# AlexandreRouma/SDRPlusPlus

Measured on NVIDIA H100. Metric: complex IQ MSamples/s through FFT + 8-VFO WFM chain, higher is better.
Workload: dtype f32

## Files before the change

sdrplusplus_b200/csrc/api.cpp:

```cpp
#include "../../include/b200dsp.h"
#include "engine.h"
#include <chrono>
#include <map>
#include <cmath>
#include <cstdio>
#include <cstring>
#include <cstdlib>
#include <algorithm>

using namespace b200;

static int g_device = -1;

static int ensure_device() {
    int n = 0;
    cudaError_t e = cudaGetDeviceCount(&n);
    if (e != cudaSuccess || n <= 0) {
        set_error("no usable CUDA device (%s): libb200dsp has no CPU fallback", e == cudaSuccess ? "0 devices" : cudaGetErrorString(e));
        cudaGetLastError();
        return B200_ENODEV;
    }
    if (g_device < 0) { g_device = 0; }
    B200_CK(cudaSetDevice(g_device));
    return 0;
// ... 170 lines not shown
    Scheduler sch_pre;
    DevBuf pp[FE_SLOTS];
    DevBuf dc_state, dc_segA, dc_segB;
    int max_eff = 0;
};

static float fe_ingest_scale(const b200_fe* fe, int fmt) {
    if (fmt == B200_FMT_CS16) { return fe->scale16; }
    if (fmt == B200_FMT_CS8) { return fe->scale8; }
    return 0.0f;
}

static int fe_alloc_fft(b200_fe* fe) {
    int rc;
    if ((rc = fe->frame.alloc((size_t)fe->fft.nz * sizeof(float2)))) { return rc; }
    long long interval = (long long)fe->fft.nz + fe->skip;
    fe->max_lines = (int)(fe->max_eff / interval) + 2;
    return fe->lines.alloc((size_t)fe->max_lines * fe->fft.size * sizeof(float));
}

extern "C" b200_fe* b200_fe_create(double samplerate, int max_chunk) {
    if (ensure_device()) { return nullptr; }
    if (samplerate <= 0 || max_chunk < 1) { set_error("bad samplerate/max_chunk"); return nullptr; }
    b200_fe* fe = new b200_fe;
    fe->fs = samplerate;
    fe->fs_eff = samplerate;
    fe->max_chunk = max_chunk;
    fe->max_eff = max_chunk;
    int lo = 0, hi = 0;
    cudaDeviceGetStreamPriorityRange(&lo, &hi);
    int pt = 2, pm = 1, pf = 0;
    if (const char* e = getenv("B200_STREAM_PRIO")) { sscanf(e, "%d,%d,%d", &pt, &pm, &pf); }
    if (const char* e = getenv("B200_FFT_SERIAL")) { fe->fft_serial = atoi(e); }
    if (const char* e = getenv("B200_FFT_CTA")) { kernels_set_fft_cta(atoi(e)); }
    auto prio = [&](int level) { int p = lo - level; return p < hi ? hi : p; };
    bool ok = cudaStreamCreateWithPriority(&fe->own_stream, cudaStreamNonBlocking, prio(pm)) == cudaSuccess &&
              cudaStreamCreateWithFlags(&fe->copy_stream, cudaStreamNonBlocking) == cudaSuccess &&
              cudaStreamCreateWithPriority(&fe->fft_stream, cudaStreamNonBlocking, prio(pf)) == cudaSuccess &&
              cudaStreamCreateWithPriority(&fe->tail_stream, cudaStreamNonBlocking, prio(pt)) == cudaSuccess &&
              cudaStreamCreateWithFlags(&fe->join_stream, cudaStreamNonBlocking) == cudaSuccess &&
              cudaEventCreateWithFlags(&fe->ev_lines_free, cudaEventDisableTiming) == cudaSuccess &&
              cudaEventCreateWithFlags(&fe->ev_fft_go, cudaEventDisableTiming) == cudaSuccess &&
              cudaEventCreateWithFlags(&fe->ev_fft_done, cudaEventDisableTiming) == cudaSuccess;
    for (int i = 0; i < FE_SLOTS && ok; i++) {
        ok = cudaEventCreateWithFlags(&fe->ev_h2d[i], cudaEventDisableTiming) == cudaSuccess &&
             cudaEventCreateWithFlags(&fe->ev_compute[i], cudaEventDisableTiming) == cudaSuccess &&
             cudaEventCreateWithFlags(&fe->ev_tail_done[i], cudaEventDisableTiming) == cudaSuccess &&
             cudaEventCreateWithFlags(&fe->ev_out[i], cudaEventDisableTiming) == cudaSuccess;
    }
    if (!ok || fe->sch.init_raw()) {
        if (ok) {} else { cuda_fail(cudaGetLastError(), "stream/event creation"); }
        b200_fe_destroy(fe);
        return nullptr;
    }
    fe->sch.stream = fe->own_stream;
    fe->sch.fuse.on = true;
    kernels_set_xd_tma_stages(2);
    kernels_set_xd_tma_diag(0);
    {
        int dev = 0, sms = 0;
        if (cudaGetDevice(&dev) == cudaSuccess && cudaDeviceGetAttribute(&sms, cudaDevAttrMultiProcessorCount, dev) == cudaSuccess && sms > 0) {
            fe->sch.sm_count = sms;
        }
    }
    if (fe->sch.enable_overlap(fe->tail_stream)) { b200_fe_destroy(fe); return nullptr; }
    return fe;
}
// ... 202 lines not shown
    if (!strcmp(key, "graphs")) { return (long long)fe->sch.graphs.size(); }
    if (!strcmp(key, "host_ns_stage1")) { return fe->sch.host_ns[0]; }
    if (!strcmp(key, "host_ns_tail")) { return fe->sch.host_ns[1]; }
    return -1;
}
extern "C" int b200_fe_set_option(b200_fe* fe, const char* key, int value) {
    if (!fe || !key) { set_error("null argument"); return B200_EINVAL; }
    if (!strcmp(key, "s1")) { fe->sch.s1_variant = value; return 0; }
    if (!strcmp(key, "overlap")) {
        if (b200_fe_vfo_count(fe) > 0) { set_error("'overlap' must be chosen before VFOs are added"); return B200_ESTATE; }
        if (cudaDeviceSynchronize() != cudaSuccess) { return cuda_fail(cudaGetLastError(), "sync"); }
        fe->sch.tail_stream = value ? fe->tail_stream : nullptr;
        return 0;
    }
    if (!strcmp(key, "pair")) { fe->sch.pair_conjugates = value != 0; return 0; }
    if (!strcmp(key, "fft_async")) { fe->fft_async = value != 0; return 0; }
    if (!strcmp(key, "s1_mt")) { kernels_set_xd_tile(value); return 0; }
    if (!strcmp(key, "s1_cps")) { kernels_set_xd_cps(value); return 0; }
    if (!strcmp(key, "s1_stages")) { kernels_set_xd_tma_stages(value); return 0; }
    if (!strcmp(key, "s1_diag")) { kernels_set_xd_tma_diag(value); return 0; }
    if (!strcmp(key, "s1_ctas")) { kernels_set_xd_tma_ctas(value); return 0; }
    if (!strcmp(key, "tails") || !strncmp(key, "ft_", 3)) {
        if (b200_fe_vfo_count(fe) > 0) { set_error("'%s' must be chosen before VFOs are added", key); return B200_ESTATE; }
        if (!strcmp(key, "tails")) { kernels_set_tail_variant(value >= 1 ? 1 : 0); fe->sch.fuse.on = value >= 2; return 0; }
        if (!strcmp(key, "ft_ob")) { fe->sch.fuse.ob_force = value; return 0; }
        if (!strcmp(key, "ft_obmax")) { fe->sch.fuse.ob_max = value; return 0; }
        if (!strcmp(key, "ft_smem_kb")) { fe->sch.fuse.smem_limit = value * 1024; return 0; }
        if (!strcmp(key, "ft_threads")) { fe->sch.fuse.threads = value; return 0; }
        if (!strcmp(key, "ft_direct")) { fe->sch.fuse.direct = value != 0; return 0; }
        if (!strcmp(key, "ft_prereg")) { fe->sch.fuse.pre_reg = value; return 0; }
        if (!strcmp(key, "ft_regall")) { fe->sch.fuse.reg_all = value != 0; return 0; }
    }
    if (!strcmp(key, "fft")) { kernels_set_fft_variant(value); return 0; }
    if (!strcmp(key, "fft_cta")) { kernels_set_fft_cta(value); return 0; }
    if (!strcmp(key, "host_direct")) { fe->host_direct = value; return 0; }
    if (!strcmp(key, "inflight")) {
        if (value < 1 || value > FE_SLOTS) { set_error("inflight: 1 ... %d", FE_SLOTS); return B200_EINVAL; }
        fe->max_inflight = value;
        return 0;
    }
    if (!strcmp(key, "fft_serial")) { fe->fft_serial = value; return 0; }
    if (!strcmp(key, "graph")) { fe->sch.graph_tails = value; if (value == 0) { fe->sch.drop_graphs(); } return 0; }
    if (!strcmp(key, "graph_max_count")) { fe->sch.graph_max_count = value; return 0; }
    if (!strcmp(key, "pdl")) { kernels_set_pdl(value); fe->sch.drop_graphs(); return 0; }
    if (!strcmp(key, "tail_split")) { fe->sch.tail_split = value; fe->sch.drop_graphs(); return 0; }
    if (!strcmp(key, "time_s1")) { fe->sch.time_s1 = value != 0; for (auto& t : fe->sch.timers) { t.used = 0; } return 0; }
    set_error("unknown option %s", key);
    return B200_EINVAL;
}

extern "C" int b200_fe_s1_stats(b200_fe* fe, double* ms_total, int* launches) {
    if (!fe || !ms_total || !launches) { set_error("null argument"); return B200_EINVAL; }
    return fe->sch.s1_stats(ms_total, launches);
}
extern "C" int b200_fe_group_stats(b200_fe* fe, int group, double* ms_total, int* launches) {
    if (!fe || !ms_total || !launches) { set_error("null argument"); return B200_EINVAL; }
    return fe->sch.group_stats(group, ms_total, launches);
}

extern "C" int b200_fe_reset(b200_fe* fe) {
    if (!fe) { set_error("null fe"); return B200_EINVAL; }
    std::lock_guard<std::mutex> lck(fe->mtx);
    B200_CK(cudaDeviceSynchronize());
    for (auto& v : fe->vfos) {
        if (v->used) { v->chain.reset_state(); }
    }
    int rc = fe->sch.reset_raw();
// ... 35 lines not shown
                v->cfg.bandwidth = v->new_bw;
            }
            v->pend_bw = false;
        }
    }
}

static int fe_fft_chunk(b200_fe* fe, const void* dptr, int fmt, int count, int* nlines) {
    *nlines = 0;
    if (!fe->fft_on) { fe->pos += (unsigned long long)count; return 0; }
    const unsigned long long pos = fe->pos, end = pos + (unsigned long long)count;
    const unsigned long long nz = (unsigned long long)fe->fft.nz, interval = nz + (unsigned long long)fe->skip;
    const int bps = bytes_per_sample(fmt);
    const float isc = fe_ingest_scale(fe, fmt);
    fe->fft.plan.in_scale = isc;
    cudaStream_t main_s = fe->sch.stream;
    const bool async = fe->fft_async || fe->sch.tail_stream != nullptr;
    float* const lines_base = fe->lines_override ? fe->lines_override : fe->lines.as<float>();
    cudaStream_t s = async ? fe->fft_stream : main_s;
    bool forked = false;
    cudaEvent_t t_fft = nullptr;
    auto fork = [&]() -> int {
        if (async && !forked) {
            B200_CK(cudaEventRecord(fe->ev_fft_go, main_s));
            B200_CK(cudaStreamWaitEvent(s, fe->ev_fft_go, 0));
            if (fe->lines_busy) { B200_CK(cudaStreamWaitEvent(s, fe->ev_lines_free, 0)); }
            trace_mark("fft start", s);
            t_fft = fe->sch.timer_begin(2, s);
            forked = true;
        }
        return 0;
    };
    int rc = 0;
    if (fe->fstart < pos) {
        const unsigned long long fend = fe->fstart + nz;
        const unsigned long long lo = pos, hi = std::min(fend, end);
        if (hi > lo) {
            if ((rc = fork())) { return rc; }
            cudaError_t e = launch_convert_cf32(dptr, fmt, fe->frame.as<float2>() + (size_t)(lo - fe->fstart), (int)(hi - lo), isc, s);
            if (e != cudaSuccess) { return cuda_fail(e, "launch_convert_cf32"); }
            fe->sch.launches++;
        }
        if (fend <= end) {
            if ((rc = fork())) { return rc; }
            int nl = 0;
            cudaError_t e = launch_fft_frame(fe->fft.plan, fe->frame.p, FMT_CF32, fe->fft.work.as<float2>(), lines_base, nullptr, s, &nl);
            if (e != cudaSuccess) { return cuda_fail(e, "launch_fft_frame"); }
            fe->sch.launches += nl;
            (*nlines)++;
            fe->fstart += interval;
        }
    }
    if (fe->fstart >= pos && fe->fstart + nz <= end) {
        int nb = (int)((end - fe->fstart - nz) / interval) + 1;
        if (*nlines + nb > fe->max_lines) { set_error("FFT line buffer overflow"); return B200_ECAP; }
        if ((rc = fork())) { return rc; }
        const char* src = (const char*)dptr + (size_t)(fe->fstart - pos) * bps;
        int nl = 0;
        cudaError_t e = launch_fft_frames(fe->fft.plan, src, fmt, fe->fft.work.as<float2>(),
                                          lines_base + (size_t)(*nlines) * fe->fft.size, nullptr, s, &nl, nb,
                                          (long long)interval * bps);
        if (e != cudaSuccess) { return cuda_fail(e, "launch_fft_frames"); }
        fe->sch.launches += nl;
        *nlines += nb;
        fe->fstart += interval * (unsigned long long)nb;
    }
    if (fe->fstart < end && fe->fstart >= pos) {
        const unsigned long long lo = fe->fstart, hi = end;
        if (hi > lo) {
            if ((rc = fork())) { return rc; }
            const char* src = (const char*)dptr + (size_t)(lo - pos) * bps;
            cudaError_t e = launch_convert_cf32(src, fmt, fe->frame.as<float2>(), (int)(hi - lo), isc, s);
            if (e != cudaSuccess) { return cuda_fail(e, "launch_convert_cf32"); }
            fe->sch.launches++;
        }
    }
    if (forked) {
        if (t_fft) { B200_CK(cudaEventRecord(t_fft, s)); }
        trace_mark("fft done", s);
        B200_CK(cudaEventRecord(fe->ev_fft_done, s));
        fe->fft_join_pending = true;
        if (fe->fft_serial && s != main_s) { B200_CK(cudaStreamWaitEvent(main_s, fe->ev_fft_done, 0)); }
    }
    fe->pos = end;
    return 0;
}

extern "C" int b200_fe_submit(b200_fe* fe, const void* iq, int count, int in_fmt, int in_mem, b200_outputs* out) {
    if (!fe || !out || (count > 0 && !iq)) { set_error("null argument"); return B200_EINVAL; }
    if (count < 0 || count > fe->max_chunk) { set_error("count %d exceeds max_chunk %d", count, fe->max_chunk); return B200_ECAP; }
    if (in_fmt < 0 || in_fmt > 2) { set_error("bad input format"); return B200_EINVAL; }
    if (fe->nsub - fe->nwait >= (unsigned long long)fe->max_inflight) { set_error("%d chunks already in flight: call b200_fe_wait", fe->max_inflight); return B200_ESTATE; }
    std::lock_guard<std::mutex> lck(fe->mtx);
    const long long hp0 = host_clock_ns();
    apply_pending(fe);
    const int slot = (int)(fe->nsub % FE_SLOTS);
    cudaStream_t s = fe->sch.stream;
    const size_t in_bytes = (size_t)count * bytes_per_sample(in_fmt);
    std::vector<Chain*> chains;
    std::vector<int> ids;
    for (size_t i = 0; i < fe->vfos.size(); i++) {
        if (fe->vfos[i]->used) { chains.push_back(&fe->vfos[i]->chain); ids.push_back((int)i); }
    }
    const int ecount = (fe->decim > 1) ? fe->pre.peek(count) : count;
    if (ecount < 0) { set_error("input decimator is not a FIR cascade"); return B200_ESTATE; }
// ... 951 lines not shown
```

sdrplusplus_b200/csrc/fft_reg.cuh:

```cuda
#pragma once

__device__ constexpr float FR_COS[16] = { 1.000000000e+00f, 9.807852804e-01f, 9.238795325e-01f, 8.314696123e-01f, 7.071067812e-01f, 5.555702330e-01f,
                                          3.826834324e-01f, 1.950903220e-01f, 0.0f, -1.950903220e-01f, -3.826834324e-01f, -5.555702330e-01f,
                                          -7.071067812e-01f, -8.314696123e-01f, -9.238795325e-01f, -9.807852804e-01f };
__device__ constexpr float FR_SIN[16] = { 0.000000000e+00f, 1.950903220e-01f, 3.826834324e-01f, 5.555702330e-01f, 7.071067812e-01f, 8.314696123e-01f,
                                          9.238795325e-01f, 9.807852804e-01f, 1.0f, 9.807852804e-01f, 9.238795325e-01f, 8.314696123e-01f,
                                          7.071067812e-01f, 5.555702330e-01f, 3.826834324e-01f, 1.950903220e-01f };

template <int R, int K>
__device__ __forceinline__ float2 fr_mul_w(float2 v) {
    constexpr int k32 = K * (32 / R);
    if constexpr (k32 == 0) { return v; }
    else if constexpr (k32 == 8) { return make_float2(v.y, -v.x); }
    else if constexpr (k32 == 4) { return make_float2((v.x + v.y) * RSQRT2, (v.y - v.x) * RSQRT2); }
    else if constexpr (k32 == 12) { return make_float2((v.y - v.x) * RSQRT2, -(v.x + v.y) * RSQRT2); }
    else {
        constexpr float c = FR_COS[k32], s = FR_SIN[k32];
        return make_float2(fmaf(v.y, s, v.x * c), fmaf(-v.x, s, v.y * c));
    }
}
template <int R, int H, int I>
__device__ __forceinline__ void fr_stage(float2 (&a)[R]) {
    constexpr int blk = I / H, j = I % H, i0 = blk * 2 * H + j;
    const float2 u = a[i0], v = a[i0 + H];
// ... 14 lines not shown
    static constexpr int n = RA * RB;
    static constexpr int TP = RA > RB ? RA : RB;
    static constexpr int crow = RB + 1;
    static constexpr int pitch = ((RA * crow + 13) / 16) * 16 + 2;
};

template <int RA, int RB>
__device__ __forceinline__ void fr_transform(float2 (&v)[RA > RB ? RA : RB], float2* ex, int t, const float2* __restrict__ tw, int twsh) {
    using G = FrGeom<RA, RB>;
    if (t < RB) {
        float2 a[RA];
#pragma unroll
        for (int i = 0; i < RA; i++) { a[i] = v[i]; }
        fr_dft<RA>(a);
#pragma unroll
        for (int c = 0; c < RA; c++) {
            float2 y = a[fr_brev<RA>(c)];
            if (c > 0) { y = cmulf(y, __ldg(tw + ((size_t)(t * c) << twsh))); }
            ex[c * G::crow + t] = y;
        }
    }
    __syncthreads();
    if (t < RA) {
        float2 b[RB];
#pragma unroll
        for (int i = 0; i < RB; i++) { b[i] = ex[t * G::crow + i]; }
        fr_dft<RB>(b);
#pragma unroll
        for (int i = 0; i < RB; i++) { v[i] = b[i]; }
    }
}

template <int FMT, int RA, int RB, int C, int MINB>
__global__ void __launch_bounds__(C * FrGeom<RA, RB>::TP, MINB) k_fftr_p1(const __grid_constant__ FftPlanDev pl, const void* __restrict__ src0,
                                                                    float2* __restrict__ work0, long long src_stride_bytes) {
    using G = FrGeom<RA, RB>;
    extern __shared__ __align__(16) float2 smem[];
    const int N2 = pl.N2;
    const void* src = reinterpret_cast<const char*>(src0) + (size_t)blockIdx.y * src_stride_bytes;
    float2* work = work0 + (size_t)blockIdx.y * pl.N;
    const int col = threadIdx.x % C, t = threadIdx.x / C;
    const int n2 = blockIdx.x * C + col;
    float2 v[G::TP];
    if (t < RB) {
#pragma unroll
        for (int a = 0; a < RA; a++) { v[a] = load_windowed<FMT>(pl, src, (a * RB + t) * N2 + n2); }
    }
    fr_transform<RA, RB>(v, smem + col * G::pitch, t, pl.tw, pl.logTW - pl.logN1);
    if (t < RA) {
        const int s = pl.logN - pl.logTW;
        const unsigned msk = (1u << s) - 1u;
#pragma unroll
        for (int d = 0; d < RB; d++) {
            const int k1 = t + RA * d;
            const unsigned e = (unsigned)k1 * (unsigned)n2;
            const float2 w = cmulf(__ldg(pl.tw + (e >> s)), __ldg(pl.tw_fine + (e & msk)));
            work[(size_t)k1 * N2 + n2] = cmulf(v[fr_brev<RB>(d)], w);
        }
    }
}

template <int RA, int RB, int R>
__global__ void __launch_bounds__(R * FrGeom<RA, RB>::TP) k_fftr_p2(const __grid_constant__ FftPlanDev pl, const float2* __restrict__ work0,
                                                                    float* __restrict__ out_db0) {
    using G = FrGeom<RA, RB>;
    extern __shared__ __align__(16) float2 smem[];
    const int N1 = pl.N1, N2 = pl.N2;
    const float2* work = work0 + (size_t)blockIdx.y * pl.N;
    float* out_db = out_db0 + (size_t)blockIdx.y * pl.N;
    const int t = threadIdx.x % G::TP, row = threadIdx.x / G::TP;
    const int r0 = blockIdx.x * R;
    float2 v[G::TP];
    if (t < RB) {
        const float2* __restrict__ p = work + (size_t)(r0 + row) * N2 + t;
#pragma unroll
        for (int a = 0; a < RA; a++) { v[a] = __ldg(p + a * RB); }
    }
    fr_transform<RA, RB>(v, smem + row * G::pitch, t, pl.tw, pl.logTW - pl.logN2);
    __syncthreads();
// ... 13 lines not shown
```

sdrplusplus_b200/csrc/kernels.cu:

```cuda
#include "kernels.cuh"
#include <unordered_map>
#include <mutex>
#include <math.h>
#include <string.h>
#include <algorithm>

template <int FMT>
__device__ __forceinline__ float2 load_iq(const void* __restrict__ p, long long i, float sc) {
    if (FMT == FMT_CF32) {
        return __ldg(reinterpret_cast<const float2*>(p) + i);
    }
    else if (FMT == FMT_CS16) {
        short2 v = __ldg(reinterpret_cast<const short2*>(p) + i);
        return make_float2((float)v.x * sc, (float)v.y * sc);
    }
    else {
        char2 v = __ldg(reinterpret_cast<const char2*>(p) + i);
        return make_float2((float)v.x * sc, (float)v.y * sc);
    }
}

template <int FMT>
__device__ __forceinline__ float2 load_x(const XdParams& p, long long i) {
    if (i >= 0) {
// ... 432 lines not shown
    }
    else if (lognb == 1) {
        const int per = n >> 1, logper = logn - 1;
        for (int t = tid; t < per * C; t += nthr) {
            int c, bi;
            if (BATCH_INNER) { c = t & (C - 1); bi = t >> logC; }
            else { bi = t & (per - 1); c = t >> logper; }
            const int base = bi * 2;
            float2 a0 = s[fft_addr<BATCH_INNER>(base + 0, c, C, pitch)];
            float2 a1 = s[fft_addr<BATCH_INNER>(base + 1, c, C, pitch)];
            s[fft_addr<BATCH_INNER>(base + 0, c, C, pitch)] = cadd(a0, a1);
            s[fft_addr<BATCH_INNER>(base + 1, c, C, pitch)] = csub(a0, a1);
        }
        __syncthreads();
    }
}

__device__ __forceinline__ int bitrev(int k, int bits) { return (int)(__brev((unsigned)k) >> (32 - bits)); }

__device__ __forceinline__ float power_db(float2 X, float normFactSq) {
    float m2 = (X.x * X.x + X.y * X.y) * normFactSq;
    float l = log2f(m2);
    if (isinf(l)) { l = copysignf(127.0f, l); }
    return l * 3.01029995663981209120f;
}

template <int FMT>
__device__ __forceinline__ float2 load_windowed(const FftPlanDev& pl, const void* __restrict__ src, int n) {
    if (n >= pl.nz) { return make_float2(0.0f, 0.0f); }
    float2 x = load_iq<FMT>(src, n, pl.in_scale);
    float w = __ldg(pl.window + n);
    return make_float2(x.x * w, x.y * w);
}

template <int FMT>
__global__ void __launch_bounds__(512) k_fft_single(const __grid_constant__ FftPlanDev pl, const void* __restrict__ src0,
                                                      float* __restrict__ out_db0, float2* __restrict__ out_raw,
                                                      long long src_stride_bytes) {
    extern __shared__ __align__(16) float2 smem[];
    const int N = pl.N;
    const void* src = reinterpret_cast<const char*>(src0) + (size_t)blockIdx.y * src_stride_bytes;
    float* out_db = out_db0 + (size_t)blockIdx.y * N;
#pragma unroll 4
    for (int i = threadIdx.x; i < N; i += blockDim.x) { smem[padf(i)] = load_windowed<FMT>(pl, src, i); }
    __syncthreads();
    fft_dif_smem<false>(smem, pl.logN, 1, N, pl.tw, pl.logTW);
    const float nf = 1.0f / ((float)N * (float)N);
    for (int k = threadIdx.x; k < N; k += blockDim.x) {
        float2 X = smem[padf(bitrev(k, pl.logN))];
        out_db[k] = power_db(X, nf);
        if (out_raw) { out_raw[k] = X; }
    }
}

template <int FMT>
__global__ void __launch_bounds__(512) k_fft_p1(const __grid_constant__ FftPlanDev pl, const void* __restrict__ src0,
                                                  float2* __restrict__ work0, int C, long long src_stride_bytes) {
    extern __shared__ __align__(16) float2 smem[];
    const int N1 = pl.N1, N2 = pl.N2;
    const void* src = reinterpret_cast<const char*>(src0) + (size_t)blockIdx.y * src_stride_bytes;
    float2* work = work0 + (size_t)blockIdx.y * pl.N;
    const int c0 = blockIdx.x * C;
#pragma unroll 4
    for (int t = threadIdx.x; t < N1 * C; t += blockDim.x) {
        int n1 = t / C, c = t - n1 * C;
        smem[padf(t)] = load_windowed<FMT>(pl, src, n1 * N2 + c0 + c);
    }
    __syncthreads();
    fft_dif_smem<true>(smem, pl.logN1, C, 0, pl.tw, pl.logTW);
    const float scale = -2.0f / (float)pl.N;
    for (int t = threadIdx.x; t < N1 * C; t += blockDim.x) {
        int k1 = t / C, c = t - k1 * C;
        float2 a = smem[padf(bitrev(k1, pl.logN1) * C + c)];
        int n2 = c0 + c;
        float sn, cs;
        sincospif((float)(k1 * n2) * scale, &sn, &cs);
        work[(size_t)k1 * N2 + n2] = cmulf(a, make_float2(cs, sn));
    }
}

__global__ void __launch_bounds__(512) k_fft_p2(const __grid_constant__ FftPlanDev pl, const float2* __restrict__ work0,
                                                  float* __restrict__ out_db0, float2* __restrict__ out_raw, int R) {
    extern __shared__ __align__(16) float2 smem[];
    const int N1 = pl.N1, N2 = pl.N2;
    const float2* work = work0 + (size_t)blockIdx.y * pl.N;
    float* out_db = out_db0 + (size_t)blockIdx.y * pl.N;
    const int pitch = N2 + 1;
    const int r0 = blockIdx.x * R;
#pragma unroll 4
    for (int t = threadIdx.x; t < R * N2; t += blockDim.x) {
        int rl = t / N2, n2 = t - rl * N2;
        smem[padf(rl * pitch + n2)] = __ldg(work + (size_t)(r0 + rl) * N2 + n2);
    }
    __syncthreads();
    fft_dif_smem<false>(smem, pl.logN2, R, pitch, pl.tw, pl.logTW);
    const float nf = 1.0f / ((float)pl.N * (float)pl.N);
    for (int t = threadIdx.x; t < R * N2; t += blockDim.x) {
        int k2 = t / R, rl = t - k2 * R;
        float2 X = smem[padf(rl * pitch + bitrev(k2, pl.logN2))];
// ... 5 lines not shown

#include "fft_reg.cuh"
#include "preproc.cuh"

template <int FMT>
__global__ void __launch_bounds__(256) k_convert(const void* __restrict__ src, float2* __restrict__ dst, int n, float sc) {
    int i = blockIdx.x * blockDim.x + threadIdx.x;
    if (i < n) { dst[i] = load_iq<FMT>(src, i, sc); }
}

__global__ void __launch_bounds__(256) k_zoom_hold(const float* __restrict__ line, const int* __restrict__ start,
                                                     const int* __restrict__ len, int out_size, float* __restrict__ out,
                                                     float* hold, float hold_speed) {
    int i = blockIdx.x * blockDim.x + threadIdx.x;
    if (i >= out_size) { return; }
    float maxVal = -INFINITY;
    const int s = start[i], l = len[i];
    for (int j = 0; j < l; j++) {
        float v = __ldg(line + s + j);
        if (v > maxVal) { maxVal = v; }
    }
    out[i] = maxVal;
    if (hold && i >= 1) {
        float d = __fsub_rn(hold[i], hold_speed);
        hold[i] = (maxVal < d) ? d : maxVal;
    }
}

static int g_smem_optin = -1;
static int g_fft_variant = 1;
void kernels_set_fft_variant(int v) { g_fft_variant = v; }
int g_xd_tma_ctas = 0;
void kernels_set_xd_tma_ctas(int v) { g_xd_tma_ctas = v; }
static int g_fft_cta = 8;
void kernels_set_fft_cta(int v) { g_fft_cta = (v == 4) ? 4 : 8; }
int kernels_max_smem_optin() {
    if (g_smem_optin < 0) {
        int dev = 0, v = 0;
        cudaGetDevice(&dev);
        cudaDeviceGetAttribute(&v, cudaDevAttrMaxSharedMemoryPerBlockOptin, dev);
        g_smem_optin = v;
    }
    return g_smem_optin;
}

template <typename K>
static cudaError_t set_smem(K kernel, size_t bytes) {
    static std::mutex mtx;
    static std::unordered_map<const void*, size_t> have;
    std::lock_guard<std::mutex> lk(mtx);
    size_t& cur = have[(const void*)kernel];
    if (bytes <= cur) { return cudaSuccess; }
    cudaError_t e = cudaFuncSetAttribute(kernel, cudaFuncAttributeMaxDynamicSharedMemorySize, (int)bytes);
    if (e == cudaSuccess) { cur = bytes; }
    return e;
}

static inline int cdiv(long long a, long long b) { return (int)((a + b - 1) / b); }

#include "chanpfb.cuh"
#include "ifnr.cuh"
#include "tails_reg.cuh"


int g_xd_cps = 0;
void kernels_set_xd_cps(int v) { g_xd_cps = v; }
int g_xd_mt_override = 0;
void kernels_set_xd_tile(int mt) { g_xd_mt_override = mt; }
// ... 443 lines not shown
    }
    dim3 grid(cdiv(p.max_out, 256), p.njobs);
    k_fir_r<<<grid, 256, 0, s>>>(p);
    return cudaGetLastError();
}
cudaError_t launch_seq(const SeqParams& p, cudaStream_t s) {
    if (p.njobs <= 0) { return cudaSuccess; }
    k_seq<<<p.njobs, 32, 0, s>>>(p);
    return cudaGetLastError();
}
cudaError_t launch_m2s(const M2SParams& p, cudaStream_t s) {
    if (p.max_n <= 0 || p.njobs <= 0) { return cudaSuccess; }
    dim3 grid(cdiv(p.max_n, 256), p.njobs);
    k_m2s<<<grid, 256, 0, s>>>(p);
    return cudaGetLastError();
}
cudaError_t launch_rxl(const RxlParams& p, cudaStream_t s) {
    if (p.max_n <= 0 || p.njobs <= 0) { return cudaSuccess; }
    dim3 grid(cdiv(p.max_n, 256), p.njobs);
    k_rxl<<<grid, 256, 0, s>>>(p);
    return cudaGetLastError();
}
cudaError_t launch_scale(const ScaleParams& p, cudaStream_t s) {
    if (p.max_n <= 0 || p.njobs <= 0) { return cudaSuccess; }
    dim3 grid(cdiv(p.max_n, 256), p.njobs);
    k_scale<<<grid, 256, 0, s>>>(p);
    return cudaGetLastError();
}
cudaError_t launch_carry(const CarryParams& p, cudaStream_t s) {
    if (p.njobs <= 0) { return cudaSuccess; }
    return launch_chain(k_carry, dim3((unsigned)p.njobs), dim3(256), 0, s, p);
}

template <int FMT>
static cudaError_t launch_fft_fmt(const FftPlanDev& pl, const void* src, float2* work, float* out_db, float2* out_raw,
                                  cudaStream_t s, int* nlaunch, int nbatch, long long src_stride_bytes) {
    cudaError_t e;
    if (pl.N1 == pl.N) {
        size_t smem = ((size_t)pl.N + (pl.N >> 4) + 2) * sizeof(float2);
        e = set_smem(k_fft_single<FMT>, smem);
        if (e != cudaSuccess) { return e; }
        int thr = pl.N / 8 < 32 ? 32 : (pl.N / 8 > 512 ? 512 : pl.N / 8);
        k_fft_single<FMT><<<dim3(1, nbatch), thr, smem, s>>>(pl, src, out_db, out_raw, src_stride_bytes);
        if (nlaunch) { (*nlaunch)++; }
        return cudaGetLastError();
    }
    if (g_fft_variant >= 1 && !out_raw && pl.tw_fine && pl.logN1 >= 8 && pl.logN1 <= 10 && pl.logN2 >= 8 && pl.logN2 <= 10) {
#define FR_P1(RA, RB, CC)                                                                                      \
        do {                                                                                                   \
            const size_t sm = (size_t)CC * FrGeom<RA, RB>::pitch * sizeof(float2);                             \
            e = set_smem(k_fftr_p1<FMT, RA, RB, CC, 2>, sm);                                                   \
            if (e != cudaSuccess) { return e; }                                                                \
            k_fftr_p1<FMT, RA, RB, CC, 2><<<dim3(pl.N2 / CC, nbatch), CC * FrGeom<RA, RB>::TP, sm, s>>>(pl, src, work, src_stride_bytes); \
        } while (0)
#define FR_P2(RA, RB, RR)                                                                                      \
        do {                                                                                                   \
            const size_t sm = (size_t)RR * FrGeom<RA, RB>::pitch * sizeof(float2);                             \
            e = set_smem(k_fftr_p2<RA, RB, RR>, sm);                                                           \
            if (e != cudaSuccess) { return e; }                                                                \
            k_fftr_p2<RA, RB, RR><<<dim3(pl.N1 / RR, nbatch), RR * FrGeom<RA, RB>::TP, sm, s>>>(pl, work, out_db); \
        } while (0)
        if (g_fft_cta == 4) {
            if (pl.logN1 == 10) { FR_P1(32, 32, 4); } else if (pl.logN1 == 9) { FR_P1(16, 32, 4); } else { FR_P1(16, 16, 4); }
        }
        else {
            if (pl.logN1 == 10) { FR_P1(32, 32, 8); } else if (pl.logN1 == 9) { FR_P1(16, 32, 8); } else { FR_P1(16, 16, 8); }
        }
        e = cudaGetLastError();
        if (e != cudaSuccess) { return e; }
        if (g_fft_cta == 4) {
            if (pl.logN2 == 10) { FR_P2(32, 32, 4); } else if (pl.logN2 == 9) { FR_P2(16, 32, 4); } else { FR_P2(16, 16, 4); }
        }
        else {
            if (pl.logN2 == 10) { FR_P2(32, 32, 8); } else if (pl.logN2 == 9) { FR_P2(16, 32, 8); } else { FR_P2(16, 16, 8); }
        }
#undef FR_P1
#undef FR_P2
        if (nlaunch) { (*nlaunch) += 2; }
        return cudaGetLastError();
    }
    int C = 16;
    while (C > 4 && (pl.N2 / C) * nbatch < 2 * num_sms()) { C >>= 1; }
    while ((size_t)pl.N1 * C * sizeof(float2) > 196608 && C > 1) { C >>= 1; }
    if (C > pl.N2) { C = pl.N2; }
    int R = 16;
    while (R > 4 && (pl.N1 / R) * nbatch < 2 * num_sms()) { R >>= 1; }
    while ((size_t)R * (pl.N2 + 1) * sizeof(float2) > 196608 && R > 1) { R >>= 1; }
    if (R > pl.N1) { R = pl.N1; }
    size_t smem1 = ((size_t)pl.N1 * C + ((size_t)pl.N1 * C >> 4) + 2) * sizeof(float2);
    size_t smem2 = ((size_t)R * (pl.N2 + 1) + ((size_t)R * (pl.N2 + 1) >> 4) + 2) * sizeof(float2);
    e = set_smem(k_fft_p1<FMT>, smem1);
    if (e != cudaSuccess) { return e; }
    e = set_smem(k_fft_p2, smem2);
    if (e != cudaSuccess) { return e; }
    const int thr1 = (pl.N1 / 8) * C >= 512 ? 512 : 256, thr2 = (pl.N2 / 8) * R >= 512 ? 512 : 256;
    k_fft_p1<FMT><<<dim3(pl.N2 / C, nbatch), thr1, smem1, s>>>(pl, src, work, C, src_stride_bytes);
    e = cudaGetLastError();
    if (e != cudaSuccess) { return e; }
    k_fft_p2<<<dim3(pl.N1 / R, nbatch), thr2, smem2, s>>>(pl, work, out_db, out_raw, R);
    if (nlaunch) { (*nlaunch) += 2; }
    return cudaGetLastError();
}

cudaError_t launch_fft_frames(const FftPlanDev& pl, const void* src, int fmt, float2* work, float* out_db,
                              float2* out_raw, cudaStream_t s, int* nlaunch, int nbatch, long long src_stride_bytes) {
    if (nbatch <= 0) { return cudaSuccess; }
    if (fmt == FMT_CF32) { return launch_fft_fmt<FMT_CF32>(pl, src, work, out_db, out_raw, s, nlaunch, nbatch, src_stride_bytes); }
    if (fmt == FMT_CS16) { return launch_fft_fmt<FMT_CS16>(pl, src, work, out_db, out_raw, s, nlaunch, nbatch, src_stride_bytes); }
    return launch_fft_fmt<FMT_CS8>(pl, src, work, out_db, out_raw, s, nlaunch, nbatch, src_stride_bytes);
}
cudaError_t launch_fft_frame(const FftPlanDev& pl, const void* src, int fmt, float2* work, float* out_db,
                             float2* out_raw, cudaStream_t s, int* nlaunch) {
    return launch_fft_frames(pl, src, fmt, work, out_db, out_raw, s, nlaunch, 1, 0);
}

cudaError_t launch_convert_cf32(const void* src, int fmt, float2* dst, int n, float scale, cudaStream_t s) {
    if (n <= 0) { return cudaSuccess; }
    int grid = cdiv(n, 256);
    if (fmt == FMT_CF32) { k_convert<FMT_CF32><<<grid, 256, 0, s>>>(src, dst, n, scale); }
    else if (fmt == FMT_CS16) { k_convert<FMT_CS16><<<grid, 256, 0, s>>>(src, dst, n, scale); }
    else { k_convert<FMT_CS8><<<grid, 256, 0, s>>>(src, dst, n, scale); }
    return cudaGetLastError();
}

__global__ void __launch_bounds__(256) k_export(const float* __restrict__ in, long long n, int type, float scalar, void* __restrict__ out) {
    const long long i = (long long)blockIdx.x * blockDim.x + threadIdx.x;
    if (i >= n) { return; }
    const float x = __ldg(in + i);
    if (type == EXP_U8) {
        const float v = __fadd_rn(__fmul_rn(x, 127.0f), 128.0f);
        reinterpret_cast<unsigned char*>(out)[i] = (unsigned char)__float2int_rz(v);
    }
    else if (type == EXP_I8) {
        float r = __fmul_rn(x, scalar);
        r = fminf(fmaxf(r, -128.0f), 127.0f);
        reinterpret_cast<signed char*>(out)[i] = (signed char)__float2int_rn(r);
    }
    else if (type == EXP_I16) {
        float r = __fmul_rn(x, scalar);
        r = fminf(fmaxf(r, -32768.0f), 32767.0f);
        reinterpret_cast<short*>(out)[i] = (short)__float2int_rn(r);
    }
    else {
        float r = __fmul_rn(x, scalar);
        r = fminf(fmaxf(r, -2147483648.0f), 2147483648.0f);
        reinterpret_cast<int*>(out)[i] = __float2int_rn(r);
// ... 46 lines not shown
```

sdrplusplus_b200/csrc/kernels.cuh:

```cuda
#pragma once
#include <cuda_runtime.h>
#include <stdint.h>

#define B200_BATCH 16

enum { FMT_CF32 = 0, FMT_CS16 = 1, FMT_CS8 = 2 };

struct XdJob {
    float2* out;
    const float2* gpad;
    unsigned long long phase0;
    unsigned long long w;
    int offset;
    int n_out;
    int T;
    const float* h;
    unsigned long long w_prev;
    int retuned;
};
struct XdParams {
    const void* in;
    const float2* hist;
    int hist_len;
    int count;
// ... 229 lines not shown
struct RxlJob { const float* in; float2* out; int n; int pad; unsigned long long phase0, w; };
struct RxlParams { int njobs; int max_n; RxlJob job[B200_BATCH]; };
cudaError_t launch_rxl(const RxlParams& p, cudaStream_t s);

struct CarryJob {
    float* dst; const float* a; const void* b;
    int h, la, lb;
    int esize;
    int bfmt;
    float scale;
};
#define CARRY_BATCH 64
struct CarryParams { int njobs; CarryJob job[CARRY_BATCH]; };

struct ChanParams {
    const float2* in;
    float2* u;
    const float* h;
    int M, P, n_out;
};
cudaError_t launch_channelizer(const ChanParams& p, float2* y, const float2* tw, cudaStream_t s, int* nlaunch);

struct FftPlanDev {
    int N, logN;
    int N1, logN1;
    int N2, logN2;
    const float2* tw;
    int TW, logTW;
    const float2* tw_fine;
    const float* window;
    float in_scale;
    int nz;
};

cudaError_t launch_xlate_decim(const XdParams& p, int fmt, int variant, cudaStream_t s, int* nlaunch);
cudaError_t launch_xd_edge(const XdParams& p, int fmt, cudaStream_t s, int* nlaunch);
cudaError_t launch_fir_c(const FirParams& p, cudaStream_t s);
cudaError_t launch_fir_reg(const FirParams& p, cudaStream_t s);
cudaError_t launch_firr_reg(const FirRParams& p, cudaStream_t s);
cudaError_t launch_poly(const PolyParams& p, cudaStream_t s);
cudaError_t launch_quad(const QuadParams& p, cudaStream_t s);
cudaError_t launch_fir_r(const FirRParams& p, cudaStream_t s);
cudaError_t launch_seq(const SeqParams& p, cudaStream_t s);
cudaError_t launch_m2s(const M2SParams& p, cudaStream_t s);
cudaError_t launch_scale(const ScaleParams& p, cudaStream_t s);
cudaError_t launch_carry(const CarryParams& p, cudaStream_t s);
cudaError_t launch_fft_frame(const FftPlanDev& pl, const void* src, int fmt, float2* work, float* out_db,
                             float2* out_raw, cudaStream_t s, int* nlaunch);
cudaError_t launch_fft_frames(const FftPlanDev& pl, const void* src, int fmt, float2* work, float* out_db,
                              float2* out_raw, cudaStream_t s, int* nlaunch, int nbatch, long long src_stride_bytes);
struct DcbParams {
    const void* in;
    float2* out;
    int fmt;
    int count;
    float in_scale;
    float rate;
    int dc_on, conj_on;
    float2* state;
    float2* segB;
    float* segA;
    int nseg;
};
cudaError_t launch_preproc(const DcbParams& p, cudaStream_t s, int* nlaunch);
cudaError_t launch_convert_cf32(const void* src, int fmt, float2* dst, int n, float scale, cudaStream_t s);
enum { EXP_U8 = 0, EXP_I8 = 1, EXP_I16 = 2, EXP_I32 = 3 };
cudaError_t launch_export(const float* in, long long n, int type, float scalar, void* out, cudaStream_t s);
cudaError_t launch_index_max(const float* in, long long n, float* out_val, cudaStream_t s);
cudaError_t launch_zoom_hold_tbl(const float* line, const int* start, const int* len, int out_size, float* out,
                                 float* hold, float hold_speed, cudaStream_t s);
int kernels_max_smem_optin();
void kernels_set_tail_variant(int v);
void kernels_set_fft_variant(int v);
void kernels_set_xd_tma_ctas(int v);
void kernels_set_fft_cta(int v);
void kernels_set_xd_tile(int mt);
void kernels_set_xd_tma_diag(int v);
void kernels_set_xd_tma_stages(int n);
void kernels_set_xd_cps(int v);
```

Before: 94840.

## Fold partial straddling FFT frame into batched FFT launch via split source

The frame that straddles the previous chunk boundary is no longer handled by a separate convert kernel plus a single-frame FFT launch. Instead, the batched FFT kernels read through a split source descriptor: samples before the chunk come from the staging buffer and the rest come directly from the chunk. The trailing partial frame for CF32 input is now staged with a device-to-device memcpy instead of a convert kernel. The fft_cta=4 option is removed. The aim is fewer launches per chunk, at the cost of extra branching in the FFT load path.

```diff
diff --git a/sdrplusplus_b200/csrc/api.cpp b/sdrplusplus_b200/csrc/api.cpp
--- a/sdrplusplus_b200/csrc/api.cpp
+++ b/sdrplusplus_b200/csrc/api.cpp
@@ -226,7 +226,6 @@
     int pt = 2, pm = 1, pf = 0;
     if (const char* e = getenv("B200_STREAM_PRIO")) { sscanf(e, "%d,%d,%d", &pt, &pm, &pf); }
     if (const char* e = getenv("B200_FFT_SERIAL")) { fe->fft_serial = atoi(e); }
-    if (const char* e = getenv("B200_FFT_CTA")) { kernels_set_fft_cta(atoi(e)); }
     auto prio = [&](int level) { int p = lo - level; return p < hi ? hi : p; };
     bool ok = cudaStreamCreateWithPriority(&fe->own_stream, cudaStreamNonBlocking, prio(pm)) == cudaSuccess &&
               cudaStreamCreateWithFlags(&fe->copy_stream, cudaStreamNonBlocking) == cudaSuccess &&
@@ -495,7 +494,6 @@
         if (!strcmp(key, "ft_regall")) { fe->sch.fuse.reg_all = value != 0; return 0; }
     }
     if (!strcmp(key, "fft")) { kernels_set_fft_variant(value); return 0; }
-    if (!strcmp(key, "fft_cta")) { kernels_set_fft_cta(value); return 0; }
     if (!strcmp(key, "host_direct")) { fe->host_direct = value; return 0; }
     if (!strcmp(key, "inflight")) {
         if (value < 1 || value > FE_SLOTS) { set_error("inflight: 1 ... %d", FE_SLOTS); return B200_EINVAL; }
@@ -597,45 +595,31 @@
         return 0;
     };
     int rc = 0;
-    if (fe->fstart < pos) {
-        const unsigned long long fend = fe->fstart + nz;
-        const unsigned long long lo = pos, hi = std::min(fend, end);
-        if (hi > lo) {
-            if ((rc = fork())) { return rc; }
-            cudaError_t e = launch_convert_cf32(dptr, fmt, fe->frame.as<float2>() + (size_t)(lo - fe->fstart), (int)(hi - lo), isc, s);
-            if (e != cudaSuccess) { return cuda_fail(e, "launch_convert_cf32"); }
-            fe->sch.launches++;
-        }
-        if (fend <= end) {
-            if ((rc = fork())) { return rc; }
-            int nl = 0;
-            cudaError_t e = launch_fft_frame(fe->fft.plan, fe->frame.p, FMT_CF32, fe->fft.work.as<float2>(), lines_base, nullptr, s, &nl);
-            if (e != cudaSuccess) { return cuda_fail(e, "launch_fft_frame"); }
-            fe->sch.launches += nl;
-            (*nlines)++;
-            fe->fstart += interval;
-        }
-    }
-    if (fe->fstart >= pos && fe->fstart + nz <= end) {
-        int nb = (int)((end - fe->fstart - nz) / interval) + 1;
-        if (*nlines + nb > fe->max_lines) { set_error("FFT line buffer overflow"); return B200_ECAP; }
+    if (fe->fstart + nz <= end) {
+        const int nb = (int)((end - fe->fstart - nz) / interval) + 1;
+        if (nb > fe->max_lines) { set_error("FFT line buffer overflow"); return B200_ECAP; }
         if ((rc = fork())) { return rc; }
-        const char* src = (const char*)dptr + (size_t)(fe->fstart - pos) * bps;
+        FftSrc src;
+        src.chunk = dptr;
+        src.stage = fe->frame.as<float2>();
+        src.off0 = (long long)fe->fstart - (long long)pos;
+        src.stride = (long long)interval;
+        src.split = fe->fstart < pos ? (int)(pos - fe->fstart) : 0;
         int nl = 0;
-        cudaError_t e = launch_fft_frames(fe->fft.plan, src, fmt, fe->fft.work.as<float2>(),
-                                          lines_base + (size_t)(*nlines) * fe->fft.size, nullptr, s, &nl, nb,
-                                          (long long)interval * bps);
+        cudaError_t e = launch_fft_frames(fe->fft.plan, src, fmt, fe->fft.work.as<float2>(), lines_base, nullptr, s, &nl, nb);
         if (e != cudaSuccess) { return cuda_fail(e, "launch_fft_frames"); }
         fe->sch.launches += nl;
-        *nlines += nb;
+        *nlines = nb;
         fe->fstart += interval * (unsigned long long)nb;
     }
-    if (fe->fstart < end && fe->fstart >= pos) {
-        const unsigned long long lo = fe->fstart, hi = end;
-        if (hi > lo) {
-            if ((rc = fork())) { return rc; }
-            const char* src = (const char*)dptr + (size_t)(lo - pos) * bps;
-            cudaError_t e = launch_convert_cf32(src, fmt, fe->frame.as<float2>(), (int)(hi - lo), isc, s);
+    const unsigned long long lo = std::max(fe->fstart, pos), hi = std::min(fe->fstart + nz, end);
+    if (hi > lo) {
+        if ((rc = fork())) { return rc; }
+        const char* src = (const char*)dptr + (size_t)(lo - pos) * bps;
+        float2* dst = fe->frame.as<float2>() + (size_t)(lo - fe->fstart);
+        if (fmt == FMT_CF32) { B200_CK(cudaMemcpyAsync(dst, src, (size_t)(hi - lo) * sizeof(float2), cudaMemcpyDeviceToDevice, s)); }
+        else {
+            cudaError_t e = launch_convert_cf32(src, fmt, dst, (int)(hi - lo), isc, s);
             if (e != cudaSuccess) { return cuda_fail(e, "launch_convert_cf32"); }
             fe->sch.launches++;
         }
diff --git a/sdrplusplus_b200/csrc/fft_reg.cuh b/sdrplusplus_b200/csrc/fft_reg.cuh
--- a/sdrplusplus_b200/csrc/fft_reg.cuh
+++ b/sdrplusplus_b200/csrc/fft_reg.cuh
@@ -70,19 +70,26 @@
 }
 
 template <int FMT, int RA, int RB, int C, int MINB>
-__global__ void __launch_bounds__(C * FrGeom<RA, RB>::TP, MINB) k_fftr_p1(const __grid_constant__ FftPlanDev pl, const void* __restrict__ src0,
-                                                                    float2* __restrict__ work0, long long src_stride_bytes) {
+__global__ void __launch_bounds__(C * FrGeom<RA, RB>::TP, MINB) k_fftr_p1(const __grid_constant__ FftPlanDev pl, const __grid_constant__ FftSrc fs,
+                                                                    float2* __restrict__ work0) {
     using G = FrGeom<RA, RB>;
     extern __shared__ __align__(16) float2 smem[];
     const int N2 = pl.N2;
-    const void* src = reinterpret_cast<const char*>(src0) + (size_t)blockIdx.y * src_stride_bytes;
     float2* work = work0 + (size_t)blockIdx.y * pl.N;
     const int col = threadIdx.x % C, t = threadIdx.x / C;
     const int n2 = blockIdx.x * C + col;
+    const long long i0 = frame_first(fs, blockIdx.y);
     float2 v[G::TP];
     if (t < RB) {
+        if (i0 >= 0) {
+            const void* src = frame_ptr<FMT>(fs, i0);
 #pragma unroll
-        for (int a = 0; a < RA; a++) { v[a] = load_windowed<FMT>(pl, src, (a * RB + t) * N2 + n2); }
+            for (int a = 0; a < RA; a++) { v[a] = load_windowed<FMT>(pl, src, (a * RB + t) * N2 + n2); }
+        }
+        else {
+#pragma unroll
+            for (int a = 0; a < RA; a++) { v[a] = load_windowed_split<FMT>(pl, fs, i0, (a * RB + t) * N2 + n2); }
+        }
     }
     fr_transform<RA, RB>(v, smem + col * G::pitch, t, pl.tw, pl.logTW - pl.logN1);
     if (t < RA) {
diff --git a/sdrplusplus_b200/csrc/kernels.cu b/sdrplusplus_b200/csrc/kernels.cu
--- a/sdrplusplus_b200/csrc/kernels.cu
+++ b/sdrplusplus_b200/csrc/kernels.cu
@@ -488,17 +488,29 @@
     float w = __ldg(pl.window + n);
     return make_float2(x.x * w, x.y * w);
 }
-
 template <int FMT>
-__global__ void __launch_bounds__(512) k_fft_single(const __grid_constant__ FftPlanDev pl, const void* __restrict__ src0,
-                                                      float* __restrict__ out_db0, float2* __restrict__ out_raw,
-                                                      long long src_stride_bytes) {
+__device__ __forceinline__ float2 load_windowed_split(const FftPlanDev& pl, const FftSrc& fs, long long i0, int n) {
+    if (n >= pl.nz) { return make_float2(0.0f, 0.0f); }
+    const long long i = i0 + n;
+    const float2 x = i >= 0 ? load_iq<FMT>(fs.chunk, i, pl.in_scale) : __ldg(fs.stage + (i + fs.split));
+    const float w = __ldg(pl.window + n);
+    return make_float2(x.x * w, x.y * w);
+}
+__device__ __forceinline__ long long frame_first(const FftSrc& fs, int j) { return fs.off0 + (long long)j * fs.stride; }
+template <int FMT>
+__device__ __forceinline__ const void* frame_ptr(const FftSrc& fs, long long i0) {
+    return reinterpret_cast<const char*>(fs.chunk) + i0 * (FMT == FMT_CF32 ? 8 : (FMT == FMT_CS16 ? 4 : 2));
+}
+
+template <int FMT>
+__global__ void __launch_bounds__(512) k_fft_single(const __grid_constant__ FftPlanDev pl, const __grid_constant__ FftSrc fs,
+                                                      float* __restrict__ out_db0, float2* __restrict__ out_raw) {
     extern __shared__ __align__(16) float2 smem[];
     const int N = pl.N;
-    const void* src = reinterpret_cast<const char*>(src0) + (size_t)blockIdx.y * src_stride_bytes;
     float* out_db = out_db0 + (size_t)blockIdx.y * N;
+    const long long i0 = frame_first(fs, blockIdx.y);
 #pragma unroll 4
-    for (int i = threadIdx.x; i < N; i += blockDim.x) { smem[padf(i)] = load_windowed<FMT>(pl, src, i); }
+    for (int i = threadIdx.x; i < N; i += blockDim.x) { smem[padf(i)] = load_windowed_split<FMT>(pl, fs, i0, i); }
     __syncthreads();
     fft_dif_smem<false>(smem, pl.logN, 1, N, pl.tw, pl.logTW);
     const float nf = 1.0f / ((float)N * (float)N);
@@ -510,17 +522,17 @@
 }
 
 template <int FMT>
-__global__ void __launch_bounds__(512) k_fft_p1(const __grid_constant__ FftPlanDev pl, const void* __restrict__ src0,
-                                                  float2* __restrict__ work0, int C, long long src_stride_bytes) {
+__global__ void __launch_bounds__(512) k_fft_p1(const __grid_constant__ FftPlanDev pl, const __grid_constant__ FftSrc fs,
+                                                  float2* __restrict__ work0, int C) {
     extern __shared__ __align__(16) float2 smem[];
     const int N1 = pl.N1, N2 = pl.N2;
-    const void* src = reinterpret_cast<const char*>(src0) + (size_t)blockIdx.y * src_stride_bytes;
     float2* work = work0 + (size_t)blockIdx.y * pl.N;
     const int c0 = blockIdx.x * C;
+    const long long i0 = frame_first(fs, blockIdx.y);
 #pragma unroll 4
     for (int t = threadIdx.x; t < N1 * C; t += blockDim.x) {
         int n1 = t / C, c = t - n1 * C;
-        smem[padf(t)] = load_windowed<FMT>(pl, src, n1 * N2 + c0 + c);
+        smem[padf(t)] = load_windowed_split<FMT>(pl, fs, i0, n1 * N2 + c0 + c);
     }
     __syncthreads();
     fft_dif_smem<true>(smem, pl.logN1, C, 0, pl.tw, pl.logTW);
@@ -592,8 +604,6 @@
 void kernels_set_fft_variant(int v) { g_fft_variant = v; }
 int g_xd_tma_ctas = 0;
 void kernels_set_xd_tma_ctas(int v) { g_xd_tma_ctas = v; }
-static int g_fft_cta = 8;
-void kernels_set_fft_cta(int v) { g_fft_cta = (v == 4) ? 4 : 8; }
 int kernels_max_smem_optin() {
     if (g_smem_optin < 0) {
         int dev = 0, v = 0;
@@ -1103,52 +1113,48 @@
     return launch_chain(k_carry, dim3((unsigned)p.njobs), dim3(256), 0, s, p);
 }
 
+#define FR_C 8
+template <int FMT, int RA, int RB>
+static cudaError_t launch_fr_p1(const FftPlanDev& pl, const FftSrc& src, float2* work, int nbatch, cudaStream_t s) {
+    const size_t sm = (size_t)FR_C * FrGeom<RA, RB>::pitch * sizeof(float2);
+    cudaError_t e = set_smem(k_fftr_p1<FMT, RA, RB, FR_C, 2>, sm);
+    if (e != cudaSuccess) { return e; }
+    k_fftr_p1<FMT, RA, RB, FR_C, 2><<<dim3(pl.N2 / FR_C, nbatch), FR_C * FrGeom<RA, RB>::TP, sm, s>>>(pl, src, work);
+    return cudaGetLastError();
+}
+template <int RA, int RB>
+static cudaError_t launch_fr_p2(const FftPlanDev& pl, const float2* work, float* out_db, int nbatch, cudaStream_t s) {
+    const size_t sm = (size_t)FR_C * FrGeom<RA, RB>::pitch * sizeof(float2);
+    cudaError_t e = set_smem(k_fftr_p2<RA, RB, FR_C>, sm);
+    if (e != cudaSuccess) { return e; }
+    k_fftr_p2<RA, RB, FR_C><<<dim3(pl.N1 / FR_C, nbatch), FR_C * FrGeom<RA, RB>::TP, sm, s>>>(pl, work, out_db);
+    return cudaGetLastError();
+}
+#undef FR_C
+
 template <int FMT>
-static cudaError_t launch_fft_fmt(const FftPlanDev& pl, const void* src, float2* work, float* out_db, float2* out_raw,
-                                  cudaStream_t s, int* nlaunch, int nbatch, long long src_stride_bytes) {
+static cudaError_t launch_fft_fmt(const FftPlanDev& pl, const FftSrc& src, float2* work, float* out_db, float2* out_raw,
+                                  cudaStream_t s, int* nlaunch, int nbatch) {
     cudaError_t e;
     if (pl.N1 == pl.N) {
         size_t smem = ((size_t)pl.N + (pl.N >> 4) + 2) * sizeof(float2);
         e = set_smem(k_fft_single<FMT>, smem);
         if (e != cudaSuccess) { return e; }
         int thr = pl.N / 8 < 32 ? 32 : (pl.N / 8 > 512 ? 512 : pl.N / 8);
-        k_fft_single<FMT><<<dim3(1, nbatch), thr, smem, s>>>(pl, src, out_db, out_raw, src_stride_bytes);
+        k_fft_single<FMT><<<dim3(1, nbatch), thr, smem, s>>>(pl, src, out_db, out_raw);
         if (nlaunch) { (*nlaunch)++; }
         return cudaGetLastError();
     }
     if (g_fft_variant >= 1 && !out_raw && pl.tw_fine && pl.logN1 >= 8 && pl.logN1 <= 10 && pl.logN2 >= 8 && pl.logN2 <= 10) {
-#define FR_P1(RA, RB, CC)                                                                                      \
-        do {                                                                                                   \
-            const size_t sm = (size_t)CC * FrGeom<RA, RB>::pitch * sizeof(float2);                             \
-            e = set_smem(k_fftr_p1<FMT, RA, RB, CC, 2>, sm);                                                   \
-            if (e != cudaSuccess) { return e; }                                                                \
-            k_fftr_p1<FMT, RA, RB, CC, 2><<<dim3(pl.N2 / CC, nbatch), CC * FrGeom<RA, RB>::TP, sm, s>>>(pl, src, work, src_stride_bytes); \
-        } while (0)
-#define FR_P2(RA, RB, RR)                                                                                      \
-        do {                                                                                                   \
-            const size_t sm = (size_t)RR * FrGeom<RA, RB>::pitch * sizeof(float2);                             \
-            e = set_smem(k_fftr_p2<RA, RB, RR>, sm);                                                           \
-            if (e != cudaSuccess) { return e; }                                                                \
-            k_fftr_p2<RA, RB, RR><<<dim3(pl.N1 / RR, nbatch), RR * FrGeom<RA, RB>::TP, sm, s>>>(pl, work, out_db); \
-        } while (0)
-        if (g_fft_cta == 4) {
-            if (pl.logN1 == 10) { FR_P1(32, 32, 4); } else if (pl.logN1 == 9) { FR_P1(16, 32, 4); } else { FR_P1(16, 16, 4); }
-        }
-        else {
-            if (pl.logN1 == 10) { FR_P1(32, 32, 8); } else if (pl.logN1 == 9) { FR_P1(16, 32, 8); } else { FR_P1(16, 16, 8); }
-        }
-        e = cudaGetLastError();
+        if (pl.logN1 == 10) { e = launch_fr_p1<FMT, 32, 32>(pl, src, work, nbatch, s); }
+        else if (pl.logN1 == 9) { e = launch_fr_p1<FMT, 16, 32>(pl, src, work, nbatch, s); }
+        else { e = launch_fr_p1<FMT, 16, 16>(pl, src, work, nbatch, s); }
         if (e != cudaSuccess) { return e; }
-        if (g_fft_cta == 4) {
-            if (pl.logN2 == 10) { FR_P2(32, 32, 4); } else if (pl.logN2 == 9) { FR_P2(16, 32, 4); } else { FR_P2(16, 16, 4); }
-        }
-        else {
-            if (pl.logN2 == 10) { FR_P2(32, 32, 8); } else if (pl.logN2 == 9) { FR_P2(16, 32, 8); } else { FR_P2(16, 16, 8); }
-        }
-#undef FR_P1
-#undef FR_P2
+        if (pl.logN2 == 10) { e = launch_fr_p2<32, 32>(pl, work, out_db, nbatch, s); }
+        else if (pl.logN2 == 9) { e = launch_fr_p2<16, 32>(pl, work, out_db, nbatch, s); }
+        else { e = launch_fr_p2<16, 16>(pl, work, out_db, nbatch, s); }
         if (nlaunch) { (*nlaunch) += 2; }
-        return cudaGetLastError();
+        return e;
     }
     int C = 16;
     while (C > 4 && (pl.N2 / C) * nbatch < 2 * num_sms()) { C >>= 1; }
@@ -1165,7 +1171,7 @@
     e = set_smem(k_fft_p2, smem2);
     if (e != cudaSuccess) { return e; }
     const int thr1 = (pl.N1 / 8) * C >= 512 ? 512 : 256, thr2 = (pl.N2 / 8) * R >= 512 ? 512 : 256;
-    k_fft_p1<FMT><<<dim3(pl.N2 / C, nbatch), thr1, smem1, s>>>(pl, src, work, C, src_stride_bytes);
+    k_fft_p1<FMT><<<dim3(pl.N2 / C, nbatch), thr1, smem1, s>>>(pl, src, work, C);
     e = cudaGetLastError();
     if (e != cudaSuccess) { return e; }
     k_fft_p2<<<dim3(pl.N1 / R, nbatch), thr2, smem2, s>>>(pl, work, out_db, out_raw, R);
@@ -1173,16 +1179,19 @@
     return cudaGetLastError();
 }
 
-cudaError_t launch_fft_frames(const FftPlanDev& pl, const void* src, int fmt, float2* work, float* out_db,
-                              float2* out_raw, cudaStream_t s, int* nlaunch, int nbatch, long long src_stride_bytes) {
+cudaError_t launch_fft_frames(const FftPlanDev& pl, const FftSrc& src, int fmt, float2* work, float* out_db,
+                              float2* out_raw, cudaStream_t s, int* nlaunch, int nbatch) {
     if (nbatch <= 0) { return cudaSuccess; }
-    if (fmt == FMT_CF32) { return launch_fft_fmt<FMT_CF32>(pl, src, work, out_db, out_raw, s, nlaunch, nbatch, src_stride_bytes); }
-    if (fmt == FMT_CS16) { return launch_fft_fmt<FMT_CS16>(pl, src, work, out_db, out_raw, s, nlaunch, nbatch, src_stride_bytes); }
-    return launch_fft_fmt<FMT_CS8>(pl, src, work, out_db, out_raw, s, nlaunch, nbatch, src_stride_bytes);
+    if (fmt == FMT_CF32) { return launch_fft_fmt<FMT_CF32>(pl, src, work, out_db, out_raw, s, nlaunch, nbatch); }
+    if (fmt == FMT_CS16) { return launch_fft_fmt<FMT_CS16>(pl, src, work, out_db, out_raw, s, nlaunch, nbatch); }
+    return launch_fft_fmt<FMT_CS8>(pl, src, work, out_db, out_raw, s, nlaunch, nbatch);
 }
 cudaError_t launch_fft_frame(const FftPlanDev& pl, const void* src, int fmt, float2* work, float* out_db,
                              float2* out_raw, cudaStream_t s, int* nlaunch) {
-    return launch_fft_frames(pl, src, fmt, work, out_db, out_raw, s, nlaunch, 1, 0);
+    FftSrc fs;
+    memset(&fs, 0, sizeof(fs));
+    fs.chunk = src;
+    return launch_fft_frames(pl, fs, fmt, work, out_db, out_raw, s, nlaunch, 1);
 }
 
 cudaError_t launch_convert_cf32(const void* src, int fmt, float2* dst, int n, float scale, cudaStream_t s) {
diff --git a/sdrplusplus_b200/csrc/kernels.cuh b/sdrplusplus_b200/csrc/kernels.cuh
--- a/sdrplusplus_b200/csrc/kernels.cuh
+++ b/sdrplusplus_b200/csrc/kernels.cuh
@@ -285,6 +285,12 @@
     float in_scale;
     int nz;
 };
+struct FftSrc {
+    const void* chunk;
+    const float2* stage;
+    long long off0, stride;
+    int split;
+};
 
 cudaError_t launch_xlate_decim(const XdParams& p, int fmt, int variant, cudaStream_t s, int* nlaunch);
 cudaError_t launch_xd_edge(const XdParams& p, int fmt, cudaStream_t s, int* nlaunch);
@@ -300,8 +306,8 @@
 cudaError_t launch_carry(const CarryParams& p, cudaStream_t s);
 cudaError_t launch_fft_frame(const FftPlanDev& pl, const void* src, int fmt, float2* work, float* out_db,
                              float2* out_raw, cudaStream_t s, int* nlaunch);
-cudaError_t launch_fft_frames(const FftPlanDev& pl, const void* src, int fmt, float2* work, float* out_db,
-                              float2* out_raw, cudaStream_t s, int* nlaunch, int nbatch, long long src_stride_bytes);
+cudaError_t launch_fft_frames(const FftPlanDev& pl, const FftSrc& src, int fmt, float2* work, float* out_db,
+                              float2* out_raw, cudaStream_t s, int* nlaunch, int nbatch);
 struct DcbParams {
     const void* in;
     float2* out;
@@ -326,7 +332,6 @@
 void kernels_set_tail_variant(int v);
 void kernels_set_fft_variant(int v);
 void kernels_set_xd_tma_ctas(int v);
-void kernels_set_fft_cta(int v);
 void kernels_set_xd_tile(int mt);
 void kernels_set_xd_tma_diag(int v);
 void kernels_set_xd_tma_stages(int n);
```

After: 95420, median of 6. Within noise of the previous version (+0.6%).
